# koszullab/instaGRAAL

Measured on AMD Instinct MI355X. Metric: MCMC moves/s (accepted+rejected) at fixed n_frags x nnz, higher is better.
Workload: dtype f32 screening tier with a rigorous bound (every column) + f64 terms (f32 inputs) for the contenders / exact i64 fixed-point sums; 1 GPU; synthetic Hi-C 50k bins / 50M contacts (149003 sub-frags), level 4, 5 neighbours, nuisance sampling off; seed=0, step=one batch of 128 moves (step_sampler calls), moves_warmup=640, parallelism=1 GPU, parameters=synthetic

## Files before the change

instagraal_amd/csrc/ig_common.cuh:

```cuda
#pragma once

#include <hip/hip_runtime.h>

#include <algorithm>
#include <atomic>
#include <cstdarg>
#include <cstdio>
#include <cstdlib>
#include <cstring>
#include <numeric>
#include <string>
#include <vector>

#include "../../include/ig_detmath.h"
#include "../../include/instagraal_hip.h"
#include "ig_ops.cuh"

#define NSLOT 25
#define NCODE 8
#define NFRESH 4
#define LGF_TAB 1024
#define SCORE_THREADS 256

static thread_local std::string g_err;
// ... 125 lines not shown
    long long* sloff;
    long long pool_cap;
    uint2* coords;
    int* loc;
    CandMeta* meta;
    ColMeta* cmeta;
    long long* part;
    long long* qpart;
    double* scores;
    MoveCtl* ctl;
    int2* sinfo;
    char* rec;
    size_t rec_stride;
    struct ScreenSum* scr;
    unsigned* scr_void;
    unsigned* scr_ub;
    unsigned* cont;
    unsigned* livecol;
    unsigned* ident;
    unsigned long long* work;
    int work_cap;
    int* slot_items;
    int* pred_list;
    int* order;
    const int* stale;
    int* tail_n;
    int* tail_ent;
    int N, M, capC, capW;
    int nseg;
    int sN, sM;
    int rot, wmask;
    unsigned long long keep;
    int ring;
};
#define PS(w) (((w) + mb.rot) & mb.wmask)
#define KEPT(w) ((int)((mb.keep >> (w)) & 1ull))
#define LW(ps) (((ps) - mb.rot) & mb.wmask)
#define P_NZ 0
#ifndef SLICE_SEG
#define SLICE_SEG 16
#endif
#define P_CNT (NSLOT * 2)
#define P_STRIDE (NSLOT * 2 + SLICE_SEG)
#define Q_Z 0
#define Q_NI (NSLOT * 2)
#define Q_NZFULL (NSLOT * 3)
// ... 201 lines not shown
    long long n_batches, n_batch_committed, n_batch_pending, n_batch_predicted;
    int up_moves, up_max_c;
    void* h_stage;
    size_t h_stage_bytes;
    int own_begin, own_end;
    int own_screened;
    unsigned long long last_stale;
    long long n_window_slots;
    int max_L, max_SL;
    int win_slots = 0;
    bool full_windows;
    int* host_max;
    struct StepHost *host_step, *host_step_dev;
    int step_seq;
    struct StepHost* pub_step;
    double* pub_scores;
    bool screen_w1;
    long long n_step_tail;
    int exact_grid;
    bool have_contacts, have_sub, have_state, have_init, have_params;
    bool init_links_inverse;
};

__host__ __device__ inline size_t rec_bytes_per_slot(int capC) { return (size_t)capC * (IG_N_TMP_STRUCT * sizeof(SlotPre) + sizeof(CandPre)); }
__device__ __forceinline__ SlotPre& pre_at(const MoveBuf& mb, int cw, int slot)
{
    const int w = cw / mb.capC, c = cw % mb.capC;
    return ((SlotPre*)(mb.rec + (size_t)w * mb.rec_stride))[c * IG_N_TMP_STRUCT + slot];
}
__device__ __forceinline__ SlotPre& pre_w(const MoveBuf& mb, int w, int i) { return ((SlotPre*)(mb.rec + (size_t)PS(w) * mb.rec_stride))[i]; }
__device__ __forceinline__ CandPre& cpre_w(const MoveBuf& mb, int w, int c)
{
    return ((CandPre*)(mb.rec + (size_t)PS(w) * mb.rec_stride + (size_t)mb.capC * IG_N_TMP_STRUCT * sizeof(SlotPre)))[c];
}
__device__ __forceinline__ CandPre& cpre_at(const MoveBuf& mb, int cw)
{
    const int w = cw / mb.capC, c = cw % mb.capC;
    return ((CandPre*)(mb.rec + (size_t)w * mb.rec_stride + (size_t)mb.capC * IG_N_TMP_STRUCT * sizeof(SlotPre)))[c];
}
```

instagraal_amd/csrc/ig_host_batch.inc:

```


static int ensure_io(ig_ctx* c, int n_moves, int max_c)
{
    const size_t need = (size_t)n_moves * (sizeof(int) + (size_t)IG_MAX_CANDIDATES * sizeof(int) + sizeof(ig_move_result));
    if (c->h_stage_bytes < need) {
        if (c->h_stage) hipHostFree(c->h_stage);
        c->h_stage = nullptr;
        c->h_stage_bytes = 0;
        const size_t want = std::max(need, (size_t)1 << 20);
        if (hipHostMalloc((void**)&c->h_stage, want, hipHostMallocDefault) == hipSuccess) c->h_stage_bytes = want;
        else (void)hipGetLastError();
    }
    if (c->results_cap < n_moves) {
        const int cap = std::max(n_moves, 8192);
        hipFree(c->d_results);
        hipFree(c->d_frags);
        DALLOC(c->d_results, (size_t)cap);
        DALLOC(c->d_frags, (size_t)cap);
        c->results_cap = cap;
    }
    if ((long long)c->cands_cap < (long long)n_moves * max_c) {
        const long long cap = std::max((long long)n_moves * max_c, 8192LL * IG_MAX_CANDIDATES);
        hipFree(c->d_cands);
        DALLOC(c->d_cands, (size_t)cap);
// ... 114 lines not shown
    const PzTab pz{c->pz_tab, c->pz_n};
    if (phase == 0 || phase == 2) {
        const int n_tw = (c->M + 31) / 32 + 1;
        if (!par_only) {
            c->touched_flip ^= 1;
            c->mb.touched = c->touched_bits + (size_t)c->touched_flip * n_tw;
        }
        if (!par_only) {
            const int mean_len0 = c->n_contigs_seen > 0 ? c->N / c->n_contigs_seen : 0;
            c->mb.nseg = mean_len0 >= 600 ? SLICE_SEG : 8;
        }
        if (!par_only) {
            TimedLaunch t(c, T_GATHER);
            hipLaunchKernelGGL(k_gather, dim3(gN), dim3(256), 0, c->stream, c->st, c->glob, c->mb, c->d_cands, c->d_frags, move0, W, max_c,
                               c->tab, c->tab_prev, c->prev_touched, force_slot, c->touched_bits + (size_t)(c->touched_flip ^ 1) * n_tw, n_tw);
        }
        if (!par_only) {
            TimedLaunch t(c, T_MUTATE);
            c->own_begin = w_begin;
            c->own_end = w_end;
            if (nW > 0) {
                const int mean_len = c->n_contigs_seen > 0 ? c->N / c->n_contigs_seen : 0;
                const int mutate_threads = mean_len >= 600 ? 1024 : (mean_len >= 150 ? 512 : 256);
                hipLaunchKernelGGL(k_mutate, dim3(NSLOT, max_c, nW), dim3(mutate_threads), 0, c->stream, c->st, c->tab, c->sub_tab, c->rowptr,
                                   c->glob, c->mb, pz, w_begin);
            }
        }
        if (force_slot < 0 && nW > 0) {
            if (!par_only) {
                TimedLaunch t(c, T_SLICE);
                hipLaunchKernelGGL(k_offsets, dim3(1), dim3(OFFSETS_THREADS), 0, c->stream, c->mb, W, w_begin, w_end, max_c);
                const int rb_auto = c->n_contigs_seen > 0
                                        ? std::min(SLICE_RB, std::max(32, (int)(2.0 * (double)c->Z / (double)c->n_contigs_seen / 2100.0)))
                                        : SLICE_RB;
                const int rb = nW == 1 ? std::max(rb_auto, 192) : rb_auto;
                const int s_share = 1, s_maxj = 1 << 20;
                if (c->mb.packed)
                    hipLaunchKernelGGL(k_slice<true>, dim3(rb, max_c + 1, nW), dim3(256), 0, c->stream, c->rowptr, c->cc, c->tab, c->glob, c->mb, c->rank,
                                       c->world, w_begin, s_share, s_maxj);
                else
                    hipLaunchKernelGGL(k_slice<false>, dim3(rb, max_c + 1, nW), dim3(256), 0, c->stream, c->rowptr, c->cc, c->tab, c->glob, c->mb, c->rank,
                                       c->world, w_begin, s_share, s_maxj);
            }
            if (par_only && nWp > 0)
                hipLaunchKernelGGL(k_rescore_prepare, dim3(NSLOT, max_c, nWp), dim3(256), 0, c->stream, c->glob, c->mb, pz, pb);
            if (nWp > 0) {
            const int s_screen = getenv("IG_SCREEN") ? atoi(getenv("IG_SCREEN")) : 1;
            const int verify = getenv("IG_SCREEN_VERIFY") ? atoi(getenv("IG_SCREEN_VERIFY")) : 0;
            const bool exact_once = c->exact_next && !par_only;
            if (exact_once) c->exact_next = false;
            const bool screen = (s_screen || verify) && phase == 2 && (W > 1 || c->screen_w1) && c->world == 1 && c->mb.packed && !exact_once;
            c->tail_fused = screen;
            if (phase == 2 && !c->tail_fused) {
                hipEventRecord(c->ev_slice, c->stream);
                hipStreamWaitEvent(c->stream2, c->ev_slice, 0);
                hipLaunchKernelGGL(k_tail, dim3(max_c, nWp), dim3(256), 0, c->stream2, c->rowptr, c->cc, c->tab, c->glob, c->mb, c->lgf_tab,
                                   g_tail_quirk, pz, pb);
                hipEventRecord(c->ev_tail, c->stream2);
            }
            int contenders_only = 0;
            if (screen) {
                const int ny = (NSLOT + 1) / 2;
                const int use_order = (!par_only && pb == w_begin && pe == w_end && nWp * max_c <= (int)OFFSETS_THREADS) ? 1 : 0;
                const int nseg = c->mb.nseg;
                const int Q = std::max(1, std::min(8, (7000 + nseg * ny * max_c * nWp - 1) / (nseg * ny * max_c * nWp)));
                {
                    TimedLaunch t(c, T_SCREEN);
                    const int tsplit = (nWp == 1 && !par_only) ? 6 : 1;
                    if (c->tail_fused)
                        hipLaunchKernelGGL(k_screen_tail, dim3(max_c * nWp * tsplit + nseg * Q * ny * max_c * nWp), dim3(SCORE_THREADS), 0, c->stream,
                                           c->screen_const, c->mb, c->mb.scr, c->mb.scr_void, c->mb.scr_ub, max_c, pb, max_c * nWp * tsplit, c->rowptr, c->cc,
                                           c->tab, c->glob, c->lgf_tab, g_tail_quirk, pz, use_order, Q, tsplit);
                    else
                        hipLaunchKernelGGL(k_screen<0>, dim3(nseg * Q, ny, max_c * nWp), dim3(SCORE_THREADS), 0, c->stream, c->screen_const,
                                           c->mb, c->mb.scr, c->mb.scr_void, c->mb.scr_ub, max_c, pb, use_order, Q);
                }
#ifdef IG_SCREEN_PROBES
                static const int s_probe = getenv("IG_SCREEN_PROBE") ? atoi(getenv("IG_SCREEN_PROBE")) : -1;
                if (s_probe >= 0) {
                    const size_t C = (size_t)c->mb.capC * c->mb.capW;
                    if (!c->probe_scr) {
                        if (dalloc(&c->probe_scr, C * NSLOT) || dalloc(&c->probe_void, 2 * C)) return;
                    }
                    hipMemsetAsync(c->probe_scr, 0, C * NSLOT * sizeof(ScreenSum), c->stream);
                    hipMemsetAsync(c->probe_void, 0, 2 * C * sizeof(unsigned), c->stream);
                    TimedLaunch tp(c, T_PROBE);
// ... 14 lines not shown
                    case 32: IG_PROBE(32); break;
                    case 512: IG_PROBE(512); break;
                    case 1024: IG_PROBE(1024); break;
                    case 2048: IG_PROBE(2048); break;
                    case 1032: IG_PROBE(1032); break;
                    case 1544: IG_PROBE(1544); break;
                    case 8192: IG_PROBE(8192); break;
                    case 8199: IG_PROBE(8199); break;
                    case 4096: IG_PROBE(4096); break;
                    case 1056: IG_PROBE(1056); break;
                    case 96: IG_PROBE(96); break;
                    case 160: IG_PROBE(160); break;
                    case 288: IG_PROBE(288); break;
                    case 480: IG_PROBE(480); break;
                    default: IG_PROBE(0); break;
                    }
#undef IG_PROBE
                }
#endif
                if (c->exact_grid <= 0) c->exact_grid = 32768;
                c->exact_grid = std::max(std::min(c->exact_grid, c->mb.work_cap), exact_grid_floor(c, max_c));
                if (!c->tail_fused) hipStreamWaitEvent(c->stream, c->ev_tail, 0);
                flush_pending_sums(c);
                hipLaunchKernelGGL(k_contend, dim3(nWp), dim3(256), 0, c->stream, c->glob, c->mb, c->mb.scr, c->mb.scr_void, c->mb.scr_ub, c->mb.cont, pb,
                                   0, c->exact_grid, EXACT_CHUNK, nWp == 1 ? 1 : 0);
                if (nWp > 1) hipLaunchKernelGGL(k_worklist, dim3(nWp), dim3(256), 0, c->stream, c->mb, c->mb.cont, pb, c->exact_grid);
                contenders_only = verify ? 0 : 1;
            }
            c->own_screened = screen ? (verify ? 2 : 1) : 0;
            TimedLaunch t(c, T_SCORE);
            const int s_eb = c->mb.nseg;
            const int s_abl = getenv("IG_ABLATE") ? atoi(getenv("IG_ABLATE")) : 0;
            if (contenders_only) {
                hipLaunchKernelGGL(k_score_list<LDS_COL_SMALL>, dim3(c->exact_grid), dim3(SCORE_THREADS), 0, c->stream, c->score_const, c->mb,
                                   c->lgf_tab, pz, s_abl, max_c, pb, 1);
            } else {
                hipLaunchKernelGGL(k_score_list<LDS_COL_SMALL>, dim3(s_eb, NSLOT, max_c * nWp), dim3(SCORE_THREADS), 0, c->stream, c->score_const,
                                   c->mb, c->lgf_tab, pz, s_abl, max_c, pb, 0);
            }
            if (screen && verify) {
                if (!c->screen_worst) {
                    if (dalloc(&c->screen_worst, 2) == 0) hipMemsetAsync(c->screen_worst, 0, 2 * sizeof(double), c->stream);
                }
                hipLaunchKernelGGL(k_screen_verify, dim3(nWp), dim3(256), 0, c->stream, c->glob, c->mb, c->mb.scr, c->mb.scr_void, c->mb.scr_ub, pb,
                                   c->screen_worst);
            }
            }
        }
    }
// ... 911 lines not shown
```

instagraal_amd/csrc/ig_host_core.inc:

```

static void free_map_buffers(ig_ctx* c);
static void flush_pending_sums(ig_ctx* c);

struct NuisWorker {
    std::thread th;
    std::mutex mu;
    std::condition_variable cv;
    std::atomic<int> state{0};
    int rc = 0;
    std::string err;
    int kind = 0;
    int move = 0;
    float p[8] = {0, 0, 0, 0, 0, 0, 0, 0};
    float mean_kb = 0;
    int n_sets = 0;
    std::thread::id tid;
};
static int nuis_step_begin_impl(ig_ctx* c, int32_t move, const float p_test[8], float mean_subfrag_kb);
static int g_nuis_async = 1;
static int nuis_chain_impl(ig_ctx* c, int32_t move, int32_t n_sets, float mean_subfrag_kb);
static int nuis_join(ig_ctx* c)
{
    NuisWorker* w = c->worker;
    if (!w || std::this_thread::get_id() == w->tid) return 0;
// ... 327 lines not shown
{
    free_window_buffers(m);
    free_slice_pool(m);
    hipFree(m.meta);
    hipFree(m.cmeta);
    hipFree(m.part);
    hipFree(m.scores);
    hipFree(m.slbound);
    hipFree(m.sloff);
    hipFree(m.qpart);
    hipFree(m.ctl);
    hipFree(m.sinfo);
    hipFree(m.rec);
    hipFree(m.scr);
    hipFree(m.scr_void);
    hipFree(m.scr_ub);
    hipFree(m.cont);
    hipFree(m.ident);
    hipFree(m.livecol);
    hipFree(m.work);
    hipFree(m.slot_items);
    hipFree(m.pred_list);
    hipFree(m.order);
    hipFree(m.tail_n);
    hipFree(m.tail_ent);
    memset((void*)&m, 0, sizeof m);
}
static void free_move_buffers(ig_ctx* c)
{
    free_movebuf(c->mb);
    hipFree(c->own_tag);
    hipFree(c->own_idx);
    c->own_tag = c->own_idx = nullptr;
    hipFree(c->batch_out);
    hipFree(c->dirty_buf);
    c->dirty_buf = nullptr;
    c->batch_out = nullptr;
}

extern "C" void ig_destroy(ig_ctx* c)
{
    if (!c) return;
    nuis_worker_stop(c);
    hipSetDevice(c->device);
    hipStreamSynchronize(c->stream);
    hipStreamSynchronize(c->stream2);
// ... 283 lines not shown
    DALLOC(m.sloff, C * SLICE_SEG);
    DALLOC(m.meta, C);
    DALLOC(m.cmeta, C * NSLOT * NCODE);
    DALLOC(m.part, C * P_STRIDE);
    DALLOC(m.qpart, C * Q_STRIDE);
    DALLOC(m.scores, C * IG_N_TMP_STRUCT);
    DALLOC(m.ctl, (size_t)capW);
    DALLOC(m.sinfo, C * NSLOT);
    m.rec_stride = rec_bytes_per_slot(capC);
    DALLOC(m.rec, m.rec_stride * (size_t)capW);
    DALLOC(m.scr, C * NSLOT);
    DALLOC(m.scr_void, C);
    DALLOC(m.scr_ub, C);
    DALLOC(m.cont, C);
    DALLOC(m.ident, C);
    HIPCK(memset_now(m.ident, 0, C * sizeof(unsigned)));
    DALLOC(m.livecol, C);
    HIPCK(memset_now(m.livecol, 0, C * sizeof(unsigned)));
    m.work_cap = (int)std::min<size_t>((size_t)1 << 20, 4 * C * NSLOT * SLICE_SEG + 4096);
    DALLOC(m.work, (size_t)m.work_cap + 32);
    DALLOC(m.slot_items, (size_t)capW * 8);
    DALLOC(m.pred_list, (size_t)capW + 8);
    HIPCK(memset_now(m.pred_list, 0, ((size_t)capW + 8) * sizeof(int)));
    DALLOC(m.order, C + (size_t)capW);
    HIPCK(memset_now(m.order, 0, (C + (size_t)capW) * sizeof(int)));
    DALLOC(m.tail_n, C);
    DALLOC(m.tail_ent, C * 3 * 64);
    HIPCK(memset_now(m.tail_n, 0xff, C * sizeof(int)));
    HIPCK(memset_now(m.cont, 0xff, C * sizeof(unsigned)));
    HIPCK(memset_now(m.cmeta, 0, C * NSLOT * NCODE * sizeof(ColMeta)));
    HIPCK(memset_now(m.slbound, 0, C * SLICE_SEG * sizeof(long long)));
    m.nseg = 8;
    HIPCK(memset_now(m.ctl, 0, (size_t)capW * sizeof(MoveCtl)));
    return 0;
}
```

instagraal_amd/csrc/ig_kernels_score.cuh:

```cuda
#pragma once


#define CW(w, c) (PS(w) * mb.capC + (c))

__device__ inline int build_uniq(int* u, bool first, int LA, int LB, const int* vf)
{
    int n = 0;
    if (first) {
        u[n++] = 0;
        u[n++] = 1;
    }
    u[n++] = 2;
    u[n++] = 3;
    if (LB != 1)
        for (int k = 4; k < 8; k++) u[n++] = k;
    if (LA != 1)
        for (int k = 8; k < 12; k++) u[n++] = k;
    for (int k = 12; k < IG_N_TMP_STRUCT; k++)
        if (!vf || vf[k - 12] != -1) u[n++] = k;
    return n;
}

__global__ void __launch_bounds__(256)
    k_gather(State st, Glob* g, MoveBuf mb, const int* __restrict__ cands_all, const int* __restrict__ frags_all, int move0, int W,
// ... 177 lines not shown
    }
    __syncthreads();
    if (t < C) {
        CandMeta* m = &mb.meta[CW(w, t)];
        int n = 0;
        int* u = m->uniq;
        for (int k = 0; k < NSLOT; k++) m->kidx[k] = -1;
        if (force_slot >= 0) {
            u[n++] = force_slot;
        } else if (t == 0) {
            n = build_uniq(u, true, m->LA, m->LB, (w == 0 && !mb.ring) ? g->valid_insert : nullptr);
        } else {
            n = build_uniq(u, false, m->LA, m->LB, sh_flags[t - 1]);
        }
        m->n_uniq = n;
        m->kidx[IG_N_TMP_STRUCT] = 0;
        for (int k = 0; k < n; k++) m->kidx[u[k]] = k + 1;
    }
}

#ifndef MUT_LDS_N
#define MUT_LDS_N 384
#endif
__device__ __forceinline__ void mutate_one(const State& st, const Tables& tab, const SubTab* __restrict__ sub,
                                           const long long* __restrict__ rowptr, Glob* g, const MoveBuf& mb, const PzTab& pz, int slot,
                                           int c, int w)
{
    const MoveCtl& mc = mb.ctl[PS(w)];
    if (c >= mc.C) return;
    const int cw = CW(w, c);
    const CandMeta& m = mb.meta[cw];
    const int k = m.kidx[slot];
    if (k < 0) return;
    const int N = mb.sN, M = mb.sM, n = m.n_loc;
    if (n > N || m.m_loc > M) return;
    int* base = mb.loc + ((size_t)(cw * NSLOT + slot) * NDYN) * N;
    __shared__ int s_loc[(NDYN + 3) * MUT_LDS_N];
    const bool in_lds = n <= MUT_LDS_N;
    int* wb = in_lds ? s_loc : base;
    const size_t ws = in_lds ? (size_t)MUT_LDS_N : (size_t)N;
    igd::Loc S;
    S.pos = wb;
    S.spos = wb + ws;
    S.cid = wb + 2 * ws;
    S.sbp = wb + 3 * ws;
    S.circ = wb + 4 * ws;
    S.prev = wb + 5 * ws;
    S.next = wb + 6 * ws;
    S.L = wb + 7 * ws;
    S.SL = wb + 8 * ws;
    S.LB = wb + 9 * ws;
    S.ori = wb + 10 * ws;
    const int* g_gid = mb.Lloc + (size_t)cw * N;
    S.gid = in_lds ? (const int*)(s_loc + 11 * MUT_LDS_N) : g_gid;
    S.lb = in_lds ? (const int*)(s_loc + 12 * MUT_LDS_N) : (mb.lbloc + (size_t)cw * N);
    S.sl = in_lds ? (const int*)(s_loc + 13 * MUT_LDS_N) : (mb.slloc + (size_t)cw * N);
    S.n = n;
    for (int x = threadIdx.x; x < n; x += blockDim.x) {
        const int f = g_gid[x];
        if (in_lds) {
// ... 120 lines not shown
    ni = wave_sum_ll(ni);
    const int wv = threadIdx.x >> 6;
    if ((threadIdx.x & 63) == 0) {
        red[0][wv] = hi;
        red[1][wv] = lo;
        red[2][wv] = ni;
    }
    __syncthreads();
    if (threadIdx.x == 0) {
        long long* q = mb.qpart + (size_t)cw * Q_STRIDE;
        long long s0 = 0, s1 = 0, s2 = 0;
        for (int v = 0; v < (int)(blockDim.x >> 6); v++) {
            s0 += red[0][v];
            s1 += red[1][v];
            s2 += red[2][v];
        }
        q[Q_Z + 2 * k] = s0;
        q[Q_Z + 2 * k + 1] = s1;
        q[Q_NI + k] = s2;
    }
    if (k == 0 && threadIdx.x < SLICE_SEG) mb.slbound[(size_t)cw * SLICE_SEG + threadIdx.x] = seg_bound[threadIdx.x];
}

__global__ void __launch_bounds__(1024) k_mutate(State st, Tables tab, const SubTab* __restrict__ sub, const long long* __restrict__ rowptr,
                                                Glob* g, MoveBuf mb, PzTab pz, int w_begin)
{
    if (KEPT(w_begin + (int)blockIdx.z)) return;
    mutate_one(st, tab, sub, rowptr, g, mb, pz, blockIdx.x, blockIdx.y, w_begin + blockIdx.z);
}

__global__ void __launch_bounds__(256) k_mutate_winners(State st, Tables tab, const SubTab* __restrict__ sub,
                                                        const long long* __restrict__ rowptr, Glob* g, MoveBuf mb, PzTab pz, int w_start,
                                                        int own_begin, int own_end, const int* __restrict__ batch_out)
{
    const int w = blockIdx.y;
    const int committed = batch_out[0], pending = batch_out[1];
    if (w >= own_begin && w < own_end) return;
    if (!((w >= w_start && w < committed) || w == pending)) return;
    const MoveCtl& mc = mb.ctl[PS(w)];
    if (blockIdx.x == 1 && mc.ch_slot == IG_N_TMP_STRUCT) return;
    mutate_one(st, tab, sub, rowptr, g, mb, pz, blockIdx.x == 0 ? IG_N_TMP_STRUCT : mc.ch_slot, mc.ch_c, w);
}

#define OFFSETS_THREADS 1024
__global__ void __launch_bounds__(OFFSETS_THREADS) k_offsets(MoveBuf mb, int W, int w_begin, int w_end, int max_c)
{
    __shared__ long long wave_tot[OFFSETS_THREADS / 64];
    __shared__ long long s_tot[IG_MAX_BATCH * IG_MAX_CANDIDATES];
    const int tid = threadIdx.x, lane = tid & 63, wv = tid >> 6;
    const int n_idx = (w_end - w_begin) * max_c;
    const bool can_order = n_idx <= IG_MAX_BATCH * IG_MAX_CANDIDATES && n_idx <= (int)OFFSETS_THREADS;
    long long my_tot = 0;
    if (can_order && tid < n_idx) {
        const int w = w_begin + tid / max_c, c = tid % max_c;
        const bool used = c < mb.ctl[PS(w)].C && !KEPT(w);
        for (int sg = 0; sg < SLICE_SEG; sg++) {
            const long long b = mb.slbound[(size_t)CW(w, c) * SLICE_SEG + sg];
            my_tot += (used && b > 0) ? b : 0;
        }
    }
    const int n = W * mb.capC * SLICE_SEG;
    const int per = (n + OFFSETS_THREADS - 1) / OFFSETS_THREADS;
    auto phys = [&](int i) -> size_t {
        const int cwl = i / SLICE_SEG;
        return (size_t)CW(cwl / mb.capC, cwl % mb.capC) * SLICE_SEG + (size_t)(i % SLICE_SEG);
    };
    auto bound_of = [&](int i) -> long long {
        const int cwl = i / SLICE_SEG;
        const int w = cwl / mb.capC, c = cwl % mb.capC;
        return (w >= w_begin && w < w_end && !KEPT(w) && c < mb.ctl[PS(w)].C) ? mb.slbound[phys(i)] : -1;
    };
    constexpr int PER_MAX = (IG_MAX_BATCH * IG_MAX_CANDIDATES * SLICE_SEG + OFFSETS_THREADS - 1) / OFFSETS_THREADS;
    long long bq[PER_MAX];
    __shared__ int s_over[IG_MAX_BATCH];
    if (tid < IG_MAX_BATCH) s_over[tid] = 0;
    long long sum = 0;
#pragma unroll
    for (int q = 0; q < PER_MAX; q++) {
        const int i = tid * per + q;
        bq[q] = (q < per && i < n) ? bound_of(i) : -1;
        sum += bq[q] > 0 ? bq[q] : 0;
    }
    long long incl = sum;
    for (int off = 1; off < 64; off <<= 1) {
        const long long o = __shfl_up(incl, off, 64);
        if (lane >= off) incl += o;
    }
    if (lane == 63) wave_tot[wv] = incl;
    __syncthreads();
    long long run = incl - sum;
    for (int q = 0; q < wv; q++) run += wave_tot[q];
#pragma unroll
    for (int q = 0; q < PER_MAX; q++) {
        const int i = tid * per + q;
        const long long b = bq[q];
        if (b >= 0) {
            if (run + b > mb.pool_cap) {
                mb.sloff[phys(i)] = -1;
                mb.ctl[PS(i / SLICE_SEG / mb.capC)].overflow = 1;
                s_over[i / SLICE_SEG / mb.capC] = 1;
            } else {
                mb.sloff[phys(i)] = run;
            }
            run += b;
        }
    }
    __syncthreads();
#pragma unroll
    for (int q = 0; q < PER_MAX; q++) {
        const int i = tid * per + q;
        if (bq[q] >= 0 && s_over[i / SLICE_SEG / mb.capC]) mb.sloff[phys(i)] = -1;
    }
    if (can_order) {
        if (tid < n_idx) s_tot[tid] = my_tot;
        __syncthreads();
        if (tid < n_idx) {
            int rank = 0;
            for (int u = 0; u < n_idx; u++) rank += (s_tot[u] > my_tot) || (s_tot[u] == my_tot && u < tid);
            mb.order[rank] = ((w_begin + tid / max_c) << 8) | (tid % max_c);
        }
        const int n_slots = w_end - w_begin;
        long long st = 0;
        if (tid < n_slots)
            for (int cc2 = 0; cc2 < max_c; cc2++) st += s_tot[tid * max_c + cc2];
        __syncthreads();
        if (tid < n_slots) s_tot[tid] = st;
        __syncthreads();
        if (tid < n_slots) {
            int rank = 0;
            for (int u = 0; u < n_slots; u++) rank += (s_tot[u] > st) || (s_tot[u] == st && u < tid);
            mb.order[mb.capC * mb.capW + rank] = w_begin + tid;
        }
    } else if (tid < w_end - w_begin) {
        mb.order[mb.capC * mb.capW + tid] = w_begin + tid;
    }
}

#define LDS_COL_CAP 4096
#define DELTA_RB 128

#ifndef SLICE_RB
#define SLICE_RB 96
#endif
#ifndef SLICE_UNROLL
#define SLICE_UNROLL 4
#endif
#ifndef SLICE_MIN_WAVES
#define SLICE_MIN_WAVES 8
#endif
template <bool PACKED>
__global__ void __launch_bounds__(256, SLICE_MIN_WAVES) k_slice(const long long* __restrict__ rowptr, const int2* __restrict__ cc, Tables tab,
                                                                 Glob* g, MoveBuf mb, int rank, int world, int w_begin, int share_rows, int max_j)
{
    const int w = mb.order[mb.capC * mb.capW + blockIdx.z];
    if (KEPT(w)) return;
    const bool shared_plane = (blockIdx.y == 0);
    const int cand_plane = (int)blockIdx.y - 1;
    __shared__ long long seg_off[IG_MAX_CANDIDATES][SLICE_SEG];
// ... 1454 lines not shown
```

instagraal_amd/csrc/ig_kernels_screen.cuh:

```cuda
#pragma once

#define SCR_KL 4.0
#define SCR_KE 4.0
#define SCR_FIX 1048576.0
#ifndef EXACT_CHUNK
#define EXACT_CHUNK 4096
#endif

struct alignas(16) ScreenConst {
    float pzc[LDS_PZ + 2];
    float slope, la, lv, d_max;
    float cy;
    float pzc_max;
    float zc_ub;
    int fast;
    int pz_n;
    const float* pz_full;
    ig_params par;
    float mean_kb;
    int pz_far_ok;
};

__device__ __forceinline__ void build_screen_const_block(const Glob* g, PzTab pz, ScreenConst* out, int which)
{
// ... 611 lines not shown
{
    __shared__ ScreenLds2 L2;
    screen_block<ABL>(sc, mb, scr, scr_void, scr_ub, max_c, w_begin, blockIdx.x % mb.nseg, blockIdx.y, blockIdx.z, L2, use_order, blockIdx.x / mb.nseg, Q);
}

__global__ void __launch_bounds__(SCORE_THREADS, SCREEN_MIN_WAVES)
    k_screen_tail(const ScreenConst* __restrict__ sc, MoveBuf mb, ScreenSum* __restrict__ scr, unsigned* __restrict__ scr_void,
                  unsigned* __restrict__ scr_ub, int max_c, int w_begin, int n_tail, const long long* __restrict__ rowptr,
                  const int2* __restrict__ cc, Tables tab, Glob* g, const double* __restrict__ lgf_tab, int tail_quirk, PzTab pz, int use_order, int Q,
                  int tsplit)
{
    __shared__ __align__(16) unsigned char lds_raw[sizeof(ScreenLds2) > sizeof(TailLds) ? sizeof(ScreenLds2) : sizeof(TailLds)];
    const int b = (int)blockIdx.x;
    if (b < n_tail) {
        const int bb = b / tsplit;
        prefinal_tail(rowptr, cc, tab, g, mb, lgf_tab, tail_quirk, pz, w_begin, bb % max_c, bb / max_c, *(TailLds*)lds_raw, b % tsplit, tsplit);
        return;
    }
    const int s = b - n_tail, ny = (NSLOT + 1) / 2, nseg = mb.nseg, nxq = nseg * Q;
    screen_block(sc, mb, scr, scr_void, scr_ub, max_c, w_begin, s % nseg, (s / nxq) % ny, s / (nxq * ny), *(ScreenLds2*)lds_raw, use_order,
                 (s % nxq) / nseg, Q);
}

__global__ void __launch_bounds__(256) k_contend(Glob* g, MoveBuf mb, const ScreenSum* __restrict__ scr, const unsigned* __restrict__ scr_void,
                                                 const unsigned* __restrict__ scr_ub, unsigned* __restrict__ cont, int w_begin, int force_all, int grid_cap, int chunk0,
                                                 int inline_worklist)
{
    __shared__ double s_lo[IG_MAX_CANDIDATES * IG_N_TMP_STRUCT], s_hi[IG_MAX_CANDIDATES * IG_N_TMP_STRUCT];
    __shared__ int s_kind[IG_MAX_CANDIDATES * IG_N_TMP_STRUCT];
    __shared__ double s_best[4];
    __shared__ unsigned s_mask[IG_MAX_CANDIDATES], s_ident[IG_MAX_CANDIDATES];
    const int w = w_begin + blockIdx.x, tid = threadIdx.x;
    if (KEPT(w)) {
        if (tid < 8) mb.slot_items[w * 8 + tid] = 0;
        return;
    }
    const MoveCtl& mc = mb.ctl[PS(w)];
    const int C = mc.C, n = C * IG_N_TMP_STRUCT;
    const ig_params p = g->par[0];
    const double log_e = IG_LOG_E_F, n_tot_pxl = g->n_tot_pxl;
    const long long z_hi = g->z_hi, z_lo = g->z_lo, n_intra = g->n_intra;
    const double cur_nz = ig_acc_to_double(g->nz_hi, g->nz_lo);
    if (tid < IG_MAX_CANDIDATES) s_mask[tid] = s_ident[tid] = 0;
    __syncthreads();
    for (int i = tid; i < n; i += blockDim.x) {
        const int c = i / IG_N_TMP_STRUCT, slot = i % IG_N_TMP_STRUCT;
        const int cw = CW(w, c);
        const CandMeta& m = mb.meta[cw];
        const int k = m.kidx[slot];
        int kind = 0;
        double lo = 0.0, hi = 0.0;
        if (k > 0) {
            const bool sup = (c == 0) && mc.superset0 && (slot >= 12);
// ... 28 lines not shown
                lo = vmin - Bd - slack;
                hi = vmax + Bd + slack;
                if ((scr_ub[cw] >> k) & 1u) {
                    lo = -1e299;
                    if (kind == 1) kind = 2;
                }
                if (!(lo == lo) || !(hi == hi) || !(__builtin_fabs(lo) < 1e300) || !(__builtin_fabs(hi) < 1e300)) kind = 3;
                else if (lo <= 0.0 && hi >= 0.0 && kind == 1) kind = 2;
            }
        }
        if (kind == 3 && force_all == 2) kind = 0;
        if (kind == 3) atomic_add_ll(&g->scr_void_cols, 1);
        s_kind[i] = kind;
        s_lo[i] = lo;
        s_hi[i] = hi;
    }
    __syncthreads();
    double best = -IG_INF;
    for (int i = tid; i < n; i += blockDim.x)
        if (s_kind[i] == 1) best = __builtin_fmax(best, s_lo[i]);
    for (int o = 32; o > 0; o >>= 1) best = __builtin_fmax(best, __shfl_down(best, o, 64));
    if ((tid & 63) == 0) s_best[tid >> 6] = best;
    __syncthreads();
    best = __builtin_fmax(__builtin_fmax(s_best[0], s_best[1]), __builtin_fmax(s_best[2], s_best[3]));
    for (int i = tid; i < n; i += blockDim.x) {
        const int kind = s_kind[i];
        if (kind == 0) continue;
        if (kind == 3 || s_hi[i] >= best) {
            const int c = i / IG_N_TMP_STRUCT, slot = i % IG_N_TMP_STRUCT;
            atomicOr(&s_mask[c], (1u << mb.meta[CW(w, c)].kidx[slot]) | 1u);
        }
    }
    __syncthreads();
    if (tid < C) {
        cont[CW(w, tid)] = s_mask[tid];
        mb.ident[CW(w, tid)] = s_ident[tid];
    }
    if (tid == 0) {
        long long tot = 0;
        for (int c = 0; c < C; c++) tot += slice_total(mb.part + (size_t)CW(w, c) * P_STRIDE) * __popc(s_mask[c] & ~s_ident[c]);
        long long ch = chunk0 > 0 ? chunk0 : EXACT_CHUNK;
        while (ch < (1LL << 40) && tot / ch + (long long)C * NSLOT * mb.nseg > grid_cap / 2) ch *= 2;
        mb.ctl[PS(w)].exact_chunk = (int)ch;
        s_kind[0] = (int)ch;
    }
    __shared__ int s_items[8];
    if (tid < 8) s_items[tid] = 0;
// ... 42 lines not shown
        const long long ch = s_kind[0];
        for (int u = tid; u < C * SLICE_SEG; u += blockDim.x) {
            const int c = u / SLICE_SEG, seg = u % SLICE_SEG;
            const int cw = CW(w, c);
            const long long n_seg = mb.part[(size_t)cw * P_STRIDE + P_CNT + seg];
            const int nch = (int)((n_seg + ch - 1) / ch);
            const unsigned mask = s_mask[c] & ~s_ident[c];
            if (!nch || !mask) continue;
            const int x = seg & 7;
            int j = atomicAdd(&wl_cnt[x], nch * __popc(mask));
            for (int q = 0; q < nch; q++) {
                unsigned m = mask;
                while (m) {
                    const int k = __ffs(m) - 1;
                    m &= m - 1;
                    mb.work[16 + 8 * (size_t)(j++) + x] =
                        ((unsigned long long)q << 32) | ((unsigned long long)cw << 12) | ((unsigned long long)k << 4) | (unsigned)seg;
                }
            }
        }
    }
}

__global__ void __launch_bounds__(256) k_worklist(MoveBuf mb, const unsigned* __restrict__ cont, int w_begin, int grid_cap)
{
    __shared__ int s_base[8], s_cnt[8], s_fit;
    const int w = w_begin + blockIdx.x, tid = threadIdx.x;
    if (KEPT(w)) return;
    if (tid < 8) {
        int base = 0;
        for (int ws = w_begin; ws < w; ws++) base += mb.slot_items[ws * 8 + tid];
        s_base[tid] = base;
        s_cnt[tid] = mb.slot_items[w * 8 + tid];
    }
    __syncthreads();
    if (tid == 0) {
        bool fit = true;
        for (int x = 0; x < 8; x++) fit &= 8LL * (s_base[x] + s_cnt[x]) <= (long long)grid_cap;
        s_fit = fit;
        if (!fit && mb.ctl[PS(w)].overflow == 0) mb.ctl[PS(w)].overflow = 2;
        for (int x = 0; x < 8; x++) {
            if (fit) atomicMax(&mb.work[x], (unsigned long long)(s_base[x] + s_cnt[x]));
            atomicMax(&mb.work[8 + x], (unsigned long long)(s_base[x] + s_cnt[x]));
        }
    }
    if (tid < 8) s_cnt[tid] = 0;
    __syncthreads();
    if (!s_fit) return;
    const int C = mb.ctl[PS(w)].C;
    const long long ch = mb.ctl[PS(w)].exact_chunk;
    for (int u = tid; u < C * SLICE_SEG; u += blockDim.x) {
        const int c = u / SLICE_SEG, seg = u % SLICE_SEG;
        const int cw = CW(w, c);
        const long long n_seg = mb.part[(size_t)cw * P_STRIDE + P_CNT + seg];
        const int nch = (int)((n_seg + ch - 1) / ch);
        const unsigned mask = cont[cw] & ~mb.ident[cw];
        if (!nch || !mask) continue;
        const int x = seg & 7;
        int j = s_base[x] + atomicAdd(&s_cnt[x], nch * __popc(mask));
        for (int q = 0; q < nch; q++) {
            unsigned m = mask;
            while (m) {
                const int k = __ffs(m) - 1;
                m &= m - 1;
                mb.work[16 + 8 * (size_t)(j++) + x] =
                    ((unsigned long long)q << 32) | ((unsigned long long)cw << 12) | ((unsigned long long)k << 4) | (unsigned)seg;
            }
        }
    }
}

__global__ void k_screen_verify(Glob* g, MoveBuf mb, const ScreenSum* __restrict__ scr, const unsigned* __restrict__ scr_void,
                                const unsigned* __restrict__ scr_ub, int w_begin, double* worst)
{
    const int w = w_begin + blockIdx.x;
    if (KEPT(w)) return;
    const MoveCtl& mc = mb.ctl[PS(w)];
    for (int i = threadIdx.x; i < mc.C * NSLOT; i += blockDim.x) {
        const int c = i / NSLOT, k = i % NSLOT;
        const int cw = CW(w, c);
        if (k == 0 || k > mb.meta[cw].n_uniq) continue;
        const unsigned vd = scr_void[cw];
        if (((vd >> k) & 1u) || (vd & 1u) || ((mb.ident[cw] >> k) & 1u)) continue;
        const long long* part = mb.part + (size_t)cw * P_STRIDE;
        const double exact = ig_acc_to_double(part[P_NZ + 2 * k] - part[P_NZ], part[P_NZ + 2 * k + 1] - part[P_NZ + 1]);
        const ScreenSum a = scr[cw * NSLOT + k], b = scr[cw * NSLOT];
        const double D = (double)(a.s_fix - b.s_fix) * (1.0 / SCR_FIX);
        const double Bd = (double)(a.b_fix + b.b_fix) * (1.0 / SCR_FIX);
        if ((scr_ub[cw] >> k) & 1u) {
            if (!(exact <= D + Bd)) g->error = 7;
            continue;
        }
// ... 50 lines not shown
```

Baseline: 51780 moves/s.

## Fuse slice offsets and worklist into last-arriving block of mutate/contend kernels

Removes the separate k_offsets and k_worklist launches. The last block to finish k_mutate and k_contend now computes the slice offsets or the batch worklist, detected with an atomic ticket counter plus release/acquire fences. The offsets scan becomes a chunked block-wide scan in reused LDS, and the worklist is built by one block using wave scans. This cuts kernel launch and serialization overhead per batch. In exchange it adds a single-block tail, a larger k_contend block (1024 threads), and grid-order changes in k_mutate.

```diff
diff --git a/instagraal_amd/csrc/ig_common.cuh b/instagraal_amd/csrc/ig_common.cuh
--- a/instagraal_amd/csrc/ig_common.cuh
+++ b/instagraal_amd/csrc/ig_common.cuh
@@ -171,6 +171,7 @@
     int work_cap;
     int* slot_items;
     int* pred_list;
+    unsigned* tickets;
     int* order;
     const int* stale;
     int* tail_n;
@@ -418,6 +419,30 @@
     bool init_links_inverse;
 };
 
+__device__ __forceinline__ bool last_arriver(unsigned* counter, unsigned total, int* s_flag)
+{
+#if defined(__HIP_DEVICE_COMPILE__)
+    asm volatile("s_waitcnt vmcnt(0)" ::: "memory");
+    __syncthreads();
+    if (threadIdx.x == 0) {
+        __builtin_amdgcn_fence(__ATOMIC_RELEASE, "agent");
+        asm volatile("s_waitcnt vmcnt(0)" ::: "memory");
+        const unsigned t = __hip_atomic_fetch_add(counter, 1u, __ATOMIC_RELAXED, __HIP_MEMORY_SCOPE_AGENT);
+        const int last = (t == total - 1u) ? 1 : 0;
+        if (last) {
+            __hip_atomic_store(counter, 0u, __ATOMIC_RELAXED, __HIP_MEMORY_SCOPE_AGENT);
+            __builtin_amdgcn_fence(__ATOMIC_ACQUIRE, "agent");
+            asm volatile("s_waitcnt vmcnt(0)" ::: "memory");
+        }
+        *s_flag = last;
+    }
+    __syncthreads();
+    return *s_flag != 0;
+#else
+    return false;
+#endif
+}
+
 __host__ __device__ inline size_t rec_bytes_per_slot(int capC) { return (size_t)capC * (IG_N_TMP_STRUCT * sizeof(SlotPre) + sizeof(CandPre)); }
 __device__ __forceinline__ SlotPre& pre_at(const MoveBuf& mb, int cw, int slot)
 {
diff --git a/instagraal_amd/csrc/ig_host_batch.inc b/instagraal_amd/csrc/ig_host_batch.inc
--- a/instagraal_amd/csrc/ig_host_batch.inc
+++ b/instagraal_amd/csrc/ig_host_batch.inc
@@ -160,14 +160,13 @@
             if (nW > 0) {
                 const int mean_len = c->n_contigs_seen > 0 ? c->N / c->n_contigs_seen : 0;
                 const int mutate_threads = mean_len >= 600 ? 1024 : (mean_len >= 150 ? 512 : 256);
-                hipLaunchKernelGGL(k_mutate, dim3(NSLOT, max_c, nW), dim3(mutate_threads), 0, c->stream, c->st, c->tab, c->sub_tab, c->rowptr,
-                                   c->glob, c->mb, pz, w_begin);
+                hipLaunchKernelGGL(k_mutate, dim3(max_c, nW, NSLOT), dim3(mutate_threads), 0, c->stream, c->st, c->tab, c->sub_tab, c->rowptr,
+                                   c->glob, c->mb, pz, w_begin, W, force_slot < 0 ? 1 : 0);
             }
         }
         if (force_slot < 0 && nW > 0) {
             if (!par_only) {
                 TimedLaunch t(c, T_SLICE);
-                hipLaunchKernelGGL(k_offsets, dim3(1), dim3(OFFSETS_THREADS), 0, c->stream, c->mb, W, w_begin, w_end, max_c);
                 const int rb_auto = c->n_contigs_seen > 0
                                         ? std::min(SLICE_RB, std::max(32, (int)(2.0 * (double)c->Z / (double)c->n_contigs_seen / 2100.0)))
                                         : SLICE_RB;
@@ -199,7 +198,7 @@
             int contenders_only = 0;
             if (screen) {
                 const int ny = (NSLOT + 1) / 2;
-                const int use_order = (!par_only && pb == w_begin && pe == w_end && nWp * max_c <= (int)OFFSETS_THREADS) ? 1 : 0;
+                const int use_order = (!par_only && pb == w_begin && pe == w_end && nWp * max_c <= OFFSETS_ORDER_MAX) ? 1 : 0;
                 const int nseg = c->mb.nseg;
                 const int Q = std::max(1, std::min(8, (7000 + nseg * ny * max_c * nWp - 1) / (nseg * ny * max_c * nWp)));
                 {
@@ -260,9 +259,8 @@
                 c->exact_grid = std::max(std::min(c->exact_grid, c->mb.work_cap), exact_grid_floor(c, max_c));
                 if (!c->tail_fused) hipStreamWaitEvent(c->stream, c->ev_tail, 0);
                 flush_pending_sums(c);
-                hipLaunchKernelGGL(k_contend, dim3(nWp), dim3(256), 0, c->stream, c->glob, c->mb, c->mb.scr, c->mb.scr_void, c->mb.scr_ub, c->mb.cont, pb,
-                                   0, c->exact_grid, EXACT_CHUNK, nWp == 1 ? 1 : 0);
-                if (nWp > 1) hipLaunchKernelGGL(k_worklist, dim3(nWp), dim3(256), 0, c->stream, c->mb, c->mb.cont, pb, c->exact_grid);
+                hipLaunchKernelGGL(k_contend, dim3(nWp), dim3(CONTEND_THREADS), 0, c->stream, c->glob, c->mb, c->mb.scr, c->mb.scr_void, c->mb.scr_ub,
+                                   c->mb.cont, pb, 0, c->exact_grid, EXACT_CHUNK, nWp == 1 ? 1 : 0, max_c);
                 contenders_only = verify ? 0 : 1;
             }
             c->own_screened = screen ? (verify ? 2 : 1) : 0;
diff --git a/instagraal_amd/csrc/ig_host_core.inc b/instagraal_amd/csrc/ig_host_core.inc
--- a/instagraal_amd/csrc/ig_host_core.inc
+++ b/instagraal_amd/csrc/ig_host_core.inc
@@ -373,6 +373,7 @@
     hipFree(m.slot_items);
     hipFree(m.pred_list);
     hipFree(m.order);
+    hipFree(m.tickets);
     hipFree(m.tail_n);
     hipFree(m.tail_ent);
     memset((void*)&m, 0, sizeof m);
@@ -702,6 +703,8 @@
     DALLOC(m.slot_items, (size_t)capW * 8);
     DALLOC(m.pred_list, (size_t)capW + 8);
     HIPCK(memset_now(m.pred_list, 0, ((size_t)capW + 8) * sizeof(int)));
+    DALLOC(m.tickets, 8);
+    HIPCK(memset_now(m.tickets, 0, 8 * sizeof(unsigned)));
     DALLOC(m.order, C + (size_t)capW);
     HIPCK(memset_now(m.order, 0, (C + (size_t)capW) * sizeof(int)));
     DALLOC(m.tail_n, C);
diff --git a/instagraal_amd/csrc/ig_kernels_score.cuh b/instagraal_amd/csrc/ig_kernels_score.cuh
--- a/instagraal_amd/csrc/ig_kernels_score.cuh
+++ b/instagraal_amd/csrc/ig_kernels_score.cuh
@@ -223,9 +223,10 @@
 #ifndef MUT_LDS_N
 #define MUT_LDS_N 384
 #endif
+#define MUT_LDS_INTS ((NDYN + 3) * MUT_LDS_N)
 __device__ __forceinline__ void mutate_one(const State& st, const Tables& tab, const SubTab* __restrict__ sub,
                                            const long long* __restrict__ rowptr, Glob* g, const MoveBuf& mb, const PzTab& pz, int slot,
-                                           int c, int w)
+                                           int c, int w, int* s_loc)
 {
     const MoveCtl& mc = mb.ctl[PS(w)];
     if (c >= mc.C) return;
@@ -236,7 +237,6 @@
     const int N = mb.sN, M = mb.sM, n = m.n_loc;
     if (n > N || m.m_loc > M) return;
     int* base = mb.loc + ((size_t)(cw * NSLOT + slot) * NDYN) * N;
-    __shared__ int s_loc[(NDYN + 3) * MUT_LDS_N];
     const bool in_lds = n <= MUT_LDS_N;
     int* wb = in_lds ? s_loc : base;
     const size_t ws = in_lds ? (size_t)MUT_LDS_N : (size_t)N;
@@ -403,104 +403,100 @@
     if (k == 0 && threadIdx.x < SLICE_SEG) mb.slbound[(size_t)cw * SLICE_SEG + threadIdx.x] = seg_bound[threadIdx.x];
 }
 
-__global__ void __launch_bounds__(1024) k_mutate(State st, Tables tab, const SubTab* __restrict__ sub, const long long* __restrict__ rowptr,
-                                                Glob* g, MoveBuf mb, PzTab pz, int w_begin)
-{
-    if (KEPT(w_begin + (int)blockIdx.z)) return;
-    mutate_one(st, tab, sub, rowptr, g, mb, pz, blockIdx.x, blockIdx.y, w_begin + blockIdx.z);
-}
-
-__global__ void __launch_bounds__(256) k_mutate_winners(State st, Tables tab, const SubTab* __restrict__ sub,
-                                                        const long long* __restrict__ rowptr, Glob* g, MoveBuf mb, PzTab pz, int w_start,
-                                                        int own_begin, int own_end, const int* __restrict__ batch_out)
-{
-    const int w = blockIdx.y;
-    const int committed = batch_out[0], pending = batch_out[1];
-    if (w >= own_begin && w < own_end) return;
-    if (!((w >= w_start && w < committed) || w == pending)) return;
-    const MoveCtl& mc = mb.ctl[PS(w)];
-    if (blockIdx.x == 1 && mc.ch_slot == IG_N_TMP_STRUCT) return;
-    mutate_one(st, tab, sub, rowptr, g, mb, pz, blockIdx.x == 0 ? IG_N_TMP_STRUCT : mc.ch_slot, mc.ch_c, w);
-}
-
-#define OFFSETS_THREADS 1024
-__global__ void __launch_bounds__(OFFSETS_THREADS) k_offsets(MoveBuf mb, int W, int w_begin, int w_end, int max_c)
-{
-    __shared__ long long wave_tot[OFFSETS_THREADS / 64];
-    __shared__ long long s_tot[IG_MAX_BATCH * IG_MAX_CANDIDATES];
-    const int tid = threadIdx.x, lane = tid & 63, wv = tid >> 6;
-    const int n_idx = (w_end - w_begin) * max_c;
-    const bool can_order = n_idx <= IG_MAX_BATCH * IG_MAX_CANDIDATES && n_idx <= (int)OFFSETS_THREADS;
-    long long my_tot = 0;
-    if (can_order && tid < n_idx) {
-        const int w = w_begin + tid / max_c, c = tid % max_c;
-        const bool used = c < mb.ctl[PS(w)].C && !KEPT(w);
-        for (int sg = 0; sg < SLICE_SEG; sg++) {
-            const long long b = mb.slbound[(size_t)CW(w, c) * SLICE_SEG + sg];
-            my_tot += (used && b > 0) ? b : 0;
-        }
-    }
+#define OFFSETS_ORDER_MAX 1024
+#ifndef OFFSETS_PER
+#define OFFSETS_PER 4
+#endif
+__device__ void slice_offsets(const MoveBuf& mb, int W, int w_begin, int w_end, int max_c, int* lds)
+{
+    static_assert((IG_MAX_BATCH * IG_MAX_CANDIDATES + 16) * 8 + (2 * IG_MAX_BATCH + 1) * 4 <= MUT_LDS_INTS * 4, "slice_offsets: LDS");
+    long long* s_tot = (long long*)lds;
+    long long* wave_tot = s_tot + IG_MAX_BATCH * IG_MAX_CANDIDATES;
+    int* s_over = (int*)(wave_tot + 16);
+    int* s_C = s_over + IG_MAX_BATCH;
+    int* s_any = s_C + IG_MAX_BATCH;
+    const int tid = threadIdx.x, nth = blockDim.x, lane = tid & 63, wv = tid >> 6, nwv = nth >> 6;
+    for (int w = tid; w < IG_MAX_BATCH; w += nth) {
+        s_over[w] = 0;
+        s_C[w] = (w >= w_begin && w < w_end && !KEPT(w)) ? mb.ctl[PS(w)].C : 0;
+    }
+    if (tid == 0) *s_any = 0;
+    __syncthreads();
     const int n = W * mb.capC * SLICE_SEG;
-    const int per = (n + OFFSETS_THREADS - 1) / OFFSETS_THREADS;
     auto phys = [&](int i) -> size_t {
         const int cwl = i / SLICE_SEG;
         return (size_t)CW(cwl / mb.capC, cwl % mb.capC) * SLICE_SEG + (size_t)(i % SLICE_SEG);
     };
     auto bound_of = [&](int i) -> long long {
         const int cwl = i / SLICE_SEG;
-        const int w = cwl / mb.capC, c = cwl % mb.capC;
-        return (w >= w_begin && w < w_end && !KEPT(w) && c < mb.ctl[PS(w)].C) ? mb.slbound[phys(i)] : -1;
+        return (cwl % mb.capC) < s_C[cwl / mb.capC] ? mb.slbound[phys(i)] : -1;
     };
-    constexpr int PER_MAX = (IG_MAX_BATCH * IG_MAX_CANDIDATES * SLICE_SEG + OFFSETS_THREADS - 1) / OFFSETS_THREADS;
-    long long bq[PER_MAX];
-    __shared__ int s_over[IG_MAX_BATCH];
-    if (tid < IG_MAX_BATCH) s_over[tid] = 0;
-    long long sum = 0;
-#pragma unroll
-    for (int q = 0; q < PER_MAX; q++) {
-        const int i = tid * per + q;
-        bq[q] = (q < per && i < n) ? bound_of(i) : -1;
-        sum += bq[q] > 0 ? bq[q] : 0;
-    }
-    long long incl = sum;
-    for (int off = 1; off < 64; off <<= 1) {
-        const long long o = __shfl_up(incl, off, 64);
-        if (lane >= off) incl += o;
-    }
-    if (lane == 63) wave_tot[wv] = incl;
-    __syncthreads();
-    long long run = incl - sum;
-    for (int q = 0; q < wv; q++) run += wave_tot[q];
-#pragma unroll
-    for (int q = 0; q < PER_MAX; q++) {
-        const int i = tid * per + q;
-        const long long b = bq[q];
-        if (b >= 0) {
-            if (run + b > mb.pool_cap) {
-                mb.sloff[phys(i)] = -1;
-                mb.ctl[PS(i / SLICE_SEG / mb.capC)].overflow = 1;
-                s_over[i / SLICE_SEG / mb.capC] = 1;
-            } else {
-                mb.sloff[phys(i)] = run;
-            }
-            run += b;
-        }
-    }
-    __syncthreads();
-#pragma unroll
-    for (int q = 0; q < PER_MAX; q++) {
-        const int i = tid * per + q;
-        if (bq[q] >= 0 && s_over[i / SLICE_SEG / mb.capC]) mb.sloff[phys(i)] = -1;
-    }
+    const int per = min(OFFSETS_PER, (n + nth - 1) / nth);
+    long long carry = 0;
+    for (int base = 0; base < n; base += nth * per) {
+        long long bq[OFFSETS_PER];
+        long long sum = 0;
+#pragma unroll
+        for (int q = 0; q < OFFSETS_PER; q++) {
+            const int i = base + tid * per + q;
+            bq[q] = (q < per && i < n) ? bound_of(i) : -1;
+            sum += bq[q] > 0 ? bq[q] : 0;
+        }
+        long long incl = sum;
+        for (int off = 1; off < 64; off <<= 1) {
+            const long long o = __shfl_up(incl, off, 64);
+            if (lane >= off) incl += o;
+        }
+        if (lane == 63) wave_tot[wv] = incl;
+        __syncthreads();
+        long long run = carry + incl - sum;
+        for (int q = 0; q < nwv; q++) {
+            const long long t = wave_tot[q];
+            if (q < wv) run += t;
+            carry += t;
+        }
+#pragma unroll
+        for (int q = 0; q < OFFSETS_PER; q++) {
+            const int i = base + tid * per + q;
+            const long long b = bq[q];
+            if (b >= 0) {
+                if (run + b > mb.pool_cap) {
+                    mb.sloff[phys(i)] = -1;
+                    mb.ctl[PS(i / SLICE_SEG / mb.capC)].overflow = 1;
+                    s_over[i / SLICE_SEG / mb.capC] = 1;
+                    *s_any = 1;
+                } else {
+                    mb.sloff[phys(i)] = run;
+                }
+                run += b;
+            }
+        }
+        __syncthreads();
+    }
+    if (*s_any) {
+        for (int i = tid; i < n; i += nth)
+            if (s_over[i / SLICE_SEG / mb.capC] && bound_of(i) >= 0) mb.sloff[phys(i)] = -1;
+    }
+    const int n_idx = (w_end - w_begin) * max_c, n_slots = w_end - w_begin;
+    const bool can_order = n_idx <= IG_MAX_BATCH * IG_MAX_CANDIDATES && n_idx <= OFFSETS_ORDER_MAX;
     if (can_order) {
-        if (tid < n_idx) s_tot[tid] = my_tot;
+        for (int u = tid; u < n_idx; u += nth) {
+            const int w = w_begin + u / max_c, c = u % max_c;
+            long long tot = 0;
+            if (c < s_C[w])
+                for (int sg = 0; sg < SLICE_SEG; sg++) {
+                    const long long b = mb.slbound[(size_t)CW(w, c) * SLICE_SEG + sg];
+                    tot += b > 0 ? b : 0;
+                }
+            s_tot[u] = tot;
+        }
         __syncthreads();
-        if (tid < n_idx) {
+        for (int v = tid; v < n_idx; v += nth) {
+            const long long my_tot = s_tot[v];
             int rank = 0;
-            for (int u = 0; u < n_idx; u++) rank += (s_tot[u] > my_tot) || (s_tot[u] == my_tot && u < tid);
-            mb.order[rank] = ((w_begin + tid / max_c) << 8) | (tid % max_c);
-        }
-        const int n_slots = w_end - w_begin;
+            for (int u = 0; u < n_idx; u++) rank += (s_tot[u] > my_tot) || (s_tot[u] == my_tot && u < v);
+            mb.order[rank] = ((w_begin + v / max_c) << 8) | (v % max_c);
+        }
         long long st = 0;
         if (tid < n_slots)
             for (int cc2 = 0; cc2 < max_c; cc2++) st += s_tot[tid * max_c + cc2];
@@ -512,9 +508,35 @@
             for (int u = 0; u < n_slots; u++) rank += (s_tot[u] > st) || (s_tot[u] == st && u < tid);
             mb.order[mb.capC * mb.capW + rank] = w_begin + tid;
         }
-    } else if (tid < w_end - w_begin) {
-        mb.order[mb.capC * mb.capW + tid] = w_begin + tid;
-    }
+    } else {
+        for (int u = tid; u < n_slots; u += nth) mb.order[mb.capC * mb.capW + u] = w_begin + u;
+    }
+}
+
+__global__ void __launch_bounds__(1024) k_mutate(State st, Tables tab, const SubTab* __restrict__ sub, const long long* __restrict__ rowptr,
+                                                Glob* g, MoveBuf mb, PzTab pz, int w_begin, int W, int offsets)
+{
+    __shared__ int s_loc[MUT_LDS_INTS];
+    __shared__ int s_last;
+    const int w = w_begin + (int)blockIdx.y;
+    if (!KEPT(w)) mutate_one(st, tab, sub, rowptr, g, mb, pz, blockIdx.z == 0 ? IG_N_TMP_STRUCT : (int)blockIdx.z - 1, blockIdx.x, w, s_loc);
+    if (blockIdx.z != 0 || !offsets) return;
+    if (!last_arriver(&mb.tickets[0], gridDim.x * gridDim.y, &s_last)) return;
+    slice_offsets(mb, W, w_begin, w_begin + (int)gridDim.y, gridDim.x, s_loc);
+}
+
+__global__ void __launch_bounds__(256) k_mutate_winners(State st, Tables tab, const SubTab* __restrict__ sub,
+                                                        const long long* __restrict__ rowptr, Glob* g, MoveBuf mb, PzTab pz, int w_start,
+                                                        int own_begin, int own_end, const int* __restrict__ batch_out)
+{
+    const int w = blockIdx.y;
+    const int committed = batch_out[0], pending = batch_out[1];
+    if (w >= own_begin && w < own_end) return;
+    if (!((w >= w_start && w < committed) || w == pending)) return;
+    const MoveCtl& mc = mb.ctl[PS(w)];
+    if (blockIdx.x == 1 && mc.ch_slot == IG_N_TMP_STRUCT) return;
+    __shared__ int s_loc[MUT_LDS_INTS];
+    mutate_one(st, tab, sub, rowptr, g, mb, pz, blockIdx.x == 0 ? IG_N_TMP_STRUCT : mc.ch_slot, mc.ch_c, w, s_loc);
 }
 
 #define LDS_COL_CAP 4096
diff --git a/instagraal_amd/csrc/ig_kernels_screen.cuh b/instagraal_amd/csrc/ig_kernels_screen.cuh
--- a/instagraal_amd/csrc/ig_kernels_screen.cuh
+++ b/instagraal_amd/csrc/ig_kernels_screen.cuh
@@ -657,13 +657,14 @@
                  (s % nxq) / nseg, Q);
 }
 
-__global__ void __launch_bounds__(256) k_contend(Glob* g, MoveBuf mb, const ScreenSum* __restrict__ scr, const unsigned* __restrict__ scr_void,
-                                                 const unsigned* __restrict__ scr_ub, unsigned* __restrict__ cont, int w_begin, int force_all, int grid_cap, int chunk0,
-                                                 int inline_worklist)
+#define CONTEND_THREADS 1024
+__device__ __forceinline__ void contend_slot(Glob* g, const MoveBuf& mb, const ScreenSum* __restrict__ scr, const unsigned* __restrict__ scr_void,
+                                             const unsigned* __restrict__ scr_ub, unsigned* __restrict__ cont, int w_begin, int force_all, int grid_cap,
+                                             int chunk0, int inline_worklist)
 {
     __shared__ double s_lo[IG_MAX_CANDIDATES * IG_N_TMP_STRUCT], s_hi[IG_MAX_CANDIDATES * IG_N_TMP_STRUCT];
     __shared__ int s_kind[IG_MAX_CANDIDATES * IG_N_TMP_STRUCT];
-    __shared__ double s_best[4];
+    __shared__ double s_best[CONTEND_THREADS / 64];
     __shared__ unsigned s_mask[IG_MAX_CANDIDATES], s_ident[IG_MAX_CANDIDATES];
     const int w = w_begin + blockIdx.x, tid = threadIdx.x;
     if (KEPT(w)) {
@@ -738,7 +739,8 @@
     for (int o = 32; o > 0; o >>= 1) best = __builtin_fmax(best, __shfl_down(best, o, 64));
     if ((tid & 63) == 0) s_best[tid >> 6] = best;
     __syncthreads();
-    best = __builtin_fmax(__builtin_fmax(s_best[0], s_best[1]), __builtin_fmax(s_best[2], s_best[3]));
+    best = s_best[0];
+    for (int v = 1; v < (int)(blockDim.x >> 6); v++) best = __builtin_fmax(best, s_best[v]);
     for (int i = tid; i < n; i += blockDim.x) {
         const int kind = s_kind[i];
         if (kind == 0) continue;
@@ -827,52 +829,108 @@
     }
 }
 
-__global__ void __launch_bounds__(256) k_worklist(MoveBuf mb, const unsigned* __restrict__ cont, int w_begin, int grid_cap)
-{
-    __shared__ int s_base[8], s_cnt[8], s_fit;
-    const int w = w_begin + blockIdx.x, tid = threadIdx.x;
-    if (KEPT(w)) return;
-    if (tid < 8) {
-        int base = 0;
-        for (int ws = w_begin; ws < w; ws++) base += mb.slot_items[ws * 8 + tid];
-        s_base[tid] = base;
-        s_cnt[tid] = mb.slot_items[w * 8 + tid];
-    }
-    __syncthreads();
-    if (tid == 0) {
-        bool fit = true;
-        for (int x = 0; x < 8; x++) fit &= 8LL * (s_base[x] + s_cnt[x]) <= (long long)grid_cap;
-        s_fit = fit;
-        if (!fit && mb.ctl[PS(w)].overflow == 0) mb.ctl[PS(w)].overflow = 2;
-        for (int x = 0; x < 8; x++) {
-            if (fit) atomicMax(&mb.work[x], (unsigned long long)(s_base[x] + s_cnt[x]));
-            atomicMax(&mb.work[8 + x], (unsigned long long)(s_base[x] + s_cnt[x]));
-        }
-    }
-    if (tid < 8) s_cnt[tid] = 0;
-    __syncthreads();
-    if (!s_fit) return;
-    const int C = mb.ctl[PS(w)].C;
-    const long long ch = mb.ctl[PS(w)].exact_chunk;
-    for (int u = tid; u < C * SLICE_SEG; u += blockDim.x) {
-        const int c = u / SLICE_SEG, seg = u % SLICE_SEG;
-        const int cw = CW(w, c);
-        const long long n_seg = mb.part[(size_t)cw * P_STRIDE + P_CNT + seg];
-        const int nch = (int)((n_seg + ch - 1) / ch);
-        const unsigned mask = cont[cw] & ~mb.ident[cw];
-        if (!nch || !mask) continue;
-        const int x = seg & 7;
-        int j = s_base[x] + atomicAdd(&s_cnt[x], nch * __popc(mask));
-        for (int q = 0; q < nch; q++) {
-            unsigned m = mask;
-            while (m) {
-                const int k = __ffs(m) - 1;
-                m &= m - 1;
-                mb.work[16 + 8 * (size_t)(j++) + x] =
-                    ((unsigned long long)q << 32) | ((unsigned long long)cw << 12) | ((unsigned long long)k << 4) | (unsigned)seg;
+__device__ void batch_worklist(const MoveBuf& mb, const unsigned* cont, int w_begin, int nW, int grid_cap, int max_c)
+{
+    static_assert(SLICE_SEG == 16 && IG_MAX_BATCH <= 64 && IG_MAX_CANDIDATES <= 16, "batch_worklist: a wave scans the slots, 32 lanes a sub-list of a slot");
+    __shared__ int s_base[IG_MAX_BATCH * 8], s_end[IG_MAX_BATCH * 8];
+    __shared__ int s_fit[IG_MAX_BATCH], s_Cn[IG_MAX_BATCH], s_chk[IG_MAX_BATCH];
+    __shared__ unsigned s_m[IG_MAX_BATCH * IG_MAX_CANDIDATES];
+    const int tid = threadIdx.x, nth = blockDim.x, lane = tid & 63, wv = tid >> 6, nwv = nth >> 6;
+    for (int s = tid; s < nW; s += nth) {
+        const int w = w_begin + s;
+        s_Cn[s] = KEPT(w) ? 0 : mb.ctl[PS(w)].C;
+        s_chk[s] = KEPT(w) ? 1 : mb.ctl[PS(w)].exact_chunk;
+        s_fit[s] = 1;
+    }
+    for (int u = tid; u < nW * 8; u += nth) s_end[u] = mb.slot_items[w_begin * 8 + u];
+    for (int u = tid; u < nW * IG_MAX_CANDIDATES; u += nth) {
+        const int w = w_begin + u / IG_MAX_CANDIDATES, c = u % IG_MAX_CANDIDATES;
+        unsigned m = 0;
+        if (!KEPT(w) && c < mb.ctl[PS(w)].C) m = cont[CW(w, c)] & ~mb.ident[CW(w, c)];
+        s_m[u] = m;
+    }
+    __syncthreads();
+    for (int x = wv; x < 8; x += nwv) {
+        const int v = lane < nW ? s_end[lane * 8 + x] : 0;
+        int incl = v;
+        for (int off = 1; off < 64; off <<= 1) {
+            const int o = __shfl_up(incl, off, 64);
+            if (lane >= off) incl += o;
+        }
+        if (lane < nW) {
+            s_base[lane * 8 + x] = incl - v;
+            s_end[lane * 8 + x] = incl;
+            if (8LL * incl > (long long)grid_cap) s_fit[lane] = 0;
+        }
+    }
+    __syncthreads();
+    for (int x = wv; x < 8; x += nwv) {
+        const bool live = lane < nW && !KEPT(w_begin + lane);
+        const int e = live ? s_end[lane * 8 + x] : 0;
+        int m_fit = (live && s_fit[lane]) ? e : 0, m_all = e;
+        for (int off = 32; off > 0; off >>= 1) {
+            m_fit = max(m_fit, __shfl_xor(m_fit, off, 64));
+            m_all = max(m_all, __shfl_xor(m_all, off, 64));
+        }
+        if (lane == 0) {
+            if (m_fit) atomicMax(&mb.work[x], (unsigned long long)m_fit);
+            if (m_all) atomicMax(&mb.work[8 + x], (unsigned long long)m_all);
+        }
+    }
+    for (int s = tid; s < nW; s += nth) {
+        const int w = w_begin + s;
+        if (!KEPT(w) && !s_fit[s] && mb.ctl[PS(w)].overflow == 0) mb.ctl[PS(w)].overflow = 2;
+    }
+    int Gp = 2;
+    while (Gp < 2 * max_c) Gp <<= 1;
+    const int total = nW * 8 * Gp;
+    for (int e0 = 0; e0 < total; e0 += nth) {
+        const int e = e0 + tid;
+        int cnt = 0, nch = 0, s = 0, x = 0, seg = 0, cw = 0;
+        unsigned mask = 0;
+        if (e < total) {
+            s = e / (8 * Gp);
+            x = (e / Gp) & 7;
+            const int h = e & (Gp - 1), c = h >> 1;
+            seg = x + 8 * (h & 1);
+            if (c < s_Cn[s] && s_fit[s]) {
+                cw = CW(w_begin + s, c);
+                const long long ch = s_chk[s];
+                const long long n_seg = mb.part[(size_t)cw * P_STRIDE + P_CNT + seg];
+                nch = (int)((n_seg + ch - 1) / ch);
+                mask = s_m[s * IG_MAX_CANDIDATES + c];
+                if (nch && mask) cnt = nch * __popc(mask);
             }
         }
-    }
+        int incl = cnt;
+        for (int off = 1; off < Gp; off <<= 1) {
+            const int o = __shfl_up(incl, off, 64);
+            if ((lane & (Gp - 1)) >= off) incl += o;
+        }
+        if (cnt) {
+            int j = s_base[s * 8 + x] + incl - cnt;
+            for (int q = 0; q < nch; q++) {
+                unsigned m = mask;
+                while (m) {
+                    const int k = __ffs(m) - 1;
+                    m &= m - 1;
+                    mb.work[16 + 8 * (size_t)(j++) + x] =
+                        ((unsigned long long)q << 32) | ((unsigned long long)cw << 12) | ((unsigned long long)k << 4) | (unsigned)seg;
+                }
+            }
+        }
+    }
+}
+
+__global__ void __launch_bounds__(CONTEND_THREADS) k_contend(Glob* g, MoveBuf mb, const ScreenSum* __restrict__ scr, const unsigned* __restrict__ scr_void,
+                                                             const unsigned* __restrict__ scr_ub, unsigned* cont, int w_begin, int force_all,
+                                                             int grid_cap, int chunk0, int inline_worklist, int max_c)
+{
+    contend_slot(g, mb, scr, scr_void, scr_ub, cont, w_begin, force_all, grid_cap, chunk0, inline_worklist);
+    if (inline_worklist) return;
+    __shared__ int s_last;
+    if (!last_arriver(&mb.tickets[1], gridDim.x, &s_last)) return;
+    batch_worklist(mb, cont, w_begin, gridDim.x, grid_cap, max_c);
 }
 
 __global__ void k_screen_verify(Glob* g, MoveBuf mb, const ScreenSum* __restrict__ scr, const unsigned* __restrict__ scr_void,
```

New measurement: 51880 moves/s (median of 5 runs). Within noise of the previous version (+0.2%).
